# david-cortes/poismf

Measured on AMD Instinct MI355X. Metric: nonzeros/sec per full A+B sweep, higher is better.
Workload: dtype f32; 1 GPU; uniform 1000000x100000, 99949803 nnz (100000000 triplets, seed 1, duplicates summed), k=50, method=pg, maxupd=10, l2=1000, step=1e-09

## Files before the change

include/poismf_hip.h:

```cpp
#ifndef POISMF_HIP_H
#define POISMF_HIP_H

#include <stdbool.h>
#include <stddef.h>

#ifdef __cplusplus
extern "C" {
#endif

#ifdef _FOR_R
  #undef USE_FLOAT
#endif
#ifndef real_t
  #ifdef USE_FLOAT
    #define real_t float
  #else
    #define real_t double
  #endif
#endif
#ifndef sparse_ix
  #ifdef _FOR_R
    #define sparse_ix int
  #else
    #define sparse_ix size_t
// ... 211 lines not shown

POISMF_HIP_API int poismf_hip_session_decisions(poismf_hip_session *s, int which, unsigned *out, size_t nrows);
POISMF_HIP_API int poismf_hip_session_decision_stats(poismf_hip_session *s, int which, unsigned long long *out);
POISMF_HIP_API int poismf_hip_factors_multiple_decisions(real_t *A, real_t *B, real_t *Bsum, real_t *Amean, real_t *Xr,
                          sparse_ix *Xr_indptr, sparse_ix *Xr_indices, int k, size_t dimA, real_t l2_reg, real_t w_mult,
                          real_t step_size, size_t niter, size_t maxupd, int method, bool limit_step, bool reuse_mean,
                          unsigned *decisions);

POISMF_HIP_API int poismf_hip_session_colsum_blocks(poismf_hip_session *s, int which);
POISMF_HIP_API int poismf_hip_session_colsum_partial(poismf_hip_session *s, int which, int b_lo, int b_hi);
POISMF_HIP_API real_t *poismf_hip_session_partials(poismf_hip_session *s);
POISMF_HIP_API void poismf_hip_session_partials_ready(poismf_hip_session *s);

POISMF_HIP_API void poismf_hip_release_cache(void);
POISMF_HIP_API size_t poismf_hip_set_device_cache_mb(size_t mb);

POISMF_HIP_API int poismf_hip_debug_row_eval(real_t *G, double *f, real_t *B, real_t *Bsum, real_t *point, real_t *Xr,
                          sparse_ix *Xr_indptr, sparse_ix *Xr_indices, int k, size_t dimA, real_t l2_reg, real_t w_mult, int which);

POISMF_HIP_API size_t poismf_hip_debug_plan(const unsigned *row_nnz, size_t nrows, int nseg, int seg, size_t k, size_t dimF, int method,
                          size_t maxupd, real_t w_mult, int limit_step, int num_cu, char *buf, size_t cap);
POISMF_HIP_API size_t poismf_hip_debug_plan_widths(const unsigned *row_nnz, size_t nrows, int nseg, int seg, size_t k, size_t dimF, int method,
                          size_t maxupd, real_t w_mult, int limit_step, int num_cu, char *buf, size_t cap);
POISMF_HIP_API int poismf_hip_debug_lane_full_width(int full);

POISMF_HIP_API size_t poismf_hip_session_nnz(poismf_hip_session *s, int which);

#ifdef __cplusplus
}
#endif
#endif
```

poismf_amd/api.py:

```python
import ctypes as C
import os

import numpy as np

from . import build as _build
from . import harness

_METHOD = {"tncg": 1, "cg": 2, "pg": 3}
_LIBS = {}


class poismf_hip_params(C.Structure):
    pass


def _params_type(c_real):
    class Params(C.Structure):
        _fields_ = [("l2_reg", c_real), ("l1_reg", c_real), ("w_mult", c_real), ("step_size", c_real),
                    ("method", C.c_int), ("limit_step", C.c_int), ("maxupd", C.c_size_t),
                    ("early_stop", C.c_int), ("reuse_prev", C.c_int)]
    return Params


EXPORTED_SYMBOLS = (
    "run_poismf", "factors_multiple", "poismf_hip_coo_to_csr_csc", "predict_multiple", "topN", "poismf_hip_session_create", "poismf_hip_session_destroy", "poismf_hip_session_A",
    "poismf_hip_session_B", "poismf_hip_session_set_factors", "poismf_hip_session_get_factors",
    "poismf_hip_half_sweep", "poismf_hip_session_profile", "poismf_hip_session_kernel_time",
    "poismf_hip_session_nnz", "poismf_hip_selftest_log", "poismf_hip_session_eval_stats",
    "poismf_hip_session_create_coo", "poismf_hip_session_stream", "poismf_hip_session_factors_dirty", "poismf_hip_session_run",
    "poismf_hip_session_set_segments", "poismf_hip_session_segment_rows", "poismf_hip_half_sweep_segment", "poismf_hip_session_plan",
    "poismf_hip_session_launch_profile", "poismf_hip_session_decisions", "poismf_hip_session_decision_stats", "poismf_hip_factors_multiple_decisions",
    "poismf_hip_session_predict", "poismf_hip_session_topn", "poismf_hip_debug_row_eval", "poismf_hip_release_cache",
    "poismf_hip_set_device_cache_mb", "poismf_hip_session_colsum_blocks", "poismf_hip_session_colsum_partial", "poismf_hip_session_partials",
    "poismf_hip_session_partials_ready", "eval_llk", "poismf_hip_session_llk", "poismf_hip_debug_plan",
    "poismf_hip_debug_plan_widths", "poismf_hip_debug_lane_full_width",
    "poismf_hip_topn_batch", "poismf_hip_session_topn_batch", "poismf_hip_topn_batch_scratch_bytes",
    "poismf_hip_rank_batch", "poismf_hip_session_rank_batch", "poismf_hip_rank_batch_scratch_bytes",
    "poismf_hip_rank_include", "poismf_hip_session_rank_include", "poismf_hip_rank_include_scratch_bytes",
    "poismf_hip_topn_include", "poismf_hip_session_topn_include", "poismf_hip_topn_include_scratch_bytes", "poismf_hip_topn_include_slice",
    "poismf_hip_topn_shared", "poismf_hip_session_topn_shared", "poismf_hip_topn_shared_scratch_bytes",
    "poismf_hip_rank_shared", "poismf_hip_session_rank_shared", "poismf_hip_rank_shared_scratch_bytes",
    "poismf_hip_topn_deep", "poismf_hip_session_topn_deep", "poismf_hip_topn_deep_scratch_bytes",
)
TOPN_BATCH_MAX_N_TOP = 128
RANK_EXCLUDED = 0xFFFFFFFF
RANK_BATCH_MAX_ROW = 65536
RANK_BATCH_BUDGET_MB = 256
RANK_INCLUDE_SLICE = 1024
RANK_INCLUDE_GROUP = 128
TOPN_NONE = 2**64 - 1
TOPN_INCLUDE_MAX_ROW = 16777216
TOPN_SHARED_MAX_CELLS = 2**24
RANK_SHARED_CHUNK_CELLS = 2**19
TOPN_DEEP_MAX_N_TOP = 1024
TOPN_DEEP_BUDGET_MB = 1024


def load_library(use_float):
# ... 269 lines not shown
    if ret:
        raise MemoryError("Could not allocate enough memory.")
    return A, (dec[:, 0] & 0xffffff).astype(np.int64), dec[:, 1].astype(np.int64), (dec[:, 0] >> 24).astype(np.int64)


def debug_row_eval(B, Bsum, point, Xr_indptr, Xr_indices, Xr, l2_reg, w_mult=1., which=0):
    use_float = B.dtype == np.float32
    _check_arrays(use_float, (B, Bsum, point, Xr), (Xr_indptr, Xr_indices))
    lib = load_library(use_float)
    k = B.shape[1]
    n = Xr_indptr.shape[0] - 1
    G = np.empty((n, k), dtype=B.dtype)
    f = np.empty(n, dtype=np.float64)
    real = C.c_float if use_float else C.c_double
    fn = lib.poismf_hip_debug_row_eval
    fn.restype = C.c_int
    fn.argtypes = [C.c_void_p] * 8 + [C.c_int, C.c_size_t, real, real, C.c_int]
    ret = fn(_ptr(G), _ptr(f), _ptr(B), _ptr(Bsum), _ptr(point), _ptr(Xr), _ptr(Xr_indptr), _ptr(Xr_indices), k, n, l2_reg, w_mult, int(which))
    if ret:
        raise MemoryError("poismf_hip_debug_row_eval failed")
    return f, G


def debug_plan(row_nnz, k, dimF, method, use_float, nseg=1, seg=-1, maxupd=1, w_mult=1., limit_step=True, num_cu=256, widths=False):
    lib = load_library(use_float)
    row_nnz = np.ascontiguousarray(row_nnz, dtype=np.uint32)
    real = C.c_float if use_float else C.c_double
    fn = lib.poismf_hip_debug_plan_widths if widths else lib.poismf_hip_debug_plan
    fn.restype = C.c_size_t
    fn.argtypes = [C.c_void_p, C.c_size_t, C.c_int, C.c_int, C.c_size_t, C.c_size_t, C.c_int, C.c_size_t, real, C.c_int, C.c_int, C.c_void_p, C.c_size_t]
    args = (_ptr(row_nnz), len(row_nnz), int(nseg), int(seg), int(k), int(dimF), _METHOD[method], int(maxupd), w_mult, int(bool(limit_step)), int(num_cu))
    buf = C.create_string_buffer(int(fn(*args, None, 0)) + 1)
    fn(*args, buf, len(buf))
    return [(name.strip(), int(rows)) for name, rows in (item.rsplit(" rows=", 1) for item in buf.value.decode().split(";") if item.strip())]


def lane_full_width(use_float, full):
    fn = load_library(use_float).poismf_hip_debug_lane_full_width
    fn.restype, fn.argtypes = C.c_int, [C.c_int]
    return bool(fn(int(bool(full))))


class PoisMF:

    def __init__(self, k=50, method="tncg", l2_reg="auto", l1_reg=0.0, niter="auto", maxupd="auto",
                 limit_step=True, initial_step=1e-7, early_stop=True, reuse_prev=False, weight_mult=1.0,
                 random_state=1, use_float=True, handle_interrupt=True, nthreads=-1):
        assert method in ("tncg", "cg", "pg")
        self.k = int(k)
        self.method = method
        self.l2_reg_, self.maxupd_, self.niter_ = harness.auto_defaults(method, self.k, l2_reg, maxupd, niter)
        assert self.k > 0 and self.niter_ >= 1 and self.maxupd_ >= 1
        assert self.l2_reg_ >= 0. and l1_reg >= 0. and initial_step > 0. and weight_mult > 0.
        self.l1_reg_ = float(l1_reg)
        self.limit_step = bool(limit_step)
        self.initial_step = float(initial_step)
        self.early_stop = bool(early_stop)
        self.reuse_prev = bool(reuse_prev)
        self.weight_mult = float(weight_mult)
        self.random_state = random_state
        self.use_float = bool(use_float)
        self.handle_interrupt = bool(handle_interrupt)
        self.nthreads_ = 1 if nthreads < 1 else int(nthreads)
# ... 754 lines not shown
```

poismf_amd/csrc/plan.hpp:

```cpp
#pragma once
#include <hip/hip_runtime.h>

#include <algorithm>
#include <cstdio>
#include <cstdlib>

#include "../../include/poismf_hip.h"
#include "row_eval.hpp"
#include "devmem.hpp"

using namespace pmf;

inline hipError_t& pmf_last_hip_error()
{
    static thread_local hipError_t e = hipSuccess;
    return e;
}
inline void pmf_report_failure()
{
    const hipError_t e = pmf_last_hip_error();
    if (e == hipSuccess || e == hipErrorOutOfMemory) fprintf(stderr, "Error: out of memory.\n");
    else fprintf(stderr, "Error: the HIP device or runtime failed (%s) -- not an out-of-memory condition; the factors are not valid.\n", hipGetErrorString(e));
}
#define HIP_TRY(expr)                                                                              \
// ... 147 lines not shown
        if (cls <= 256) return { 2, 0, 0, 2, 1 };
        if (cls <= 512) return { 2, 0, 0, 4, 1 };
        if (cls <= 1024) return { 2, 0, 0, 8, 1 };
        if (cls <= 1536) return { 3, 0, 0, 8, 1 };
    }
    return { 0, 0, 0, 0, 0 };
}

#ifndef PMF_LANE_KU50
#if (defined(PMF_LANE_XPOSE) && PMF_LANE_XPOSE != 2) || (defined(PMF_LANE_COAL) && PMF_LANE_COAL == 0) || (defined(PMF_LANE_SPOINT) && PMF_LANE_SPOINT == 0) || \
    (defined(PMF_LANE_PK) && PMF_LANE_PK == 0) || (defined(PMF_LANE_PK_DOTS) && PMF_LANE_PK_DOTS == 0) || (defined(PMF_LANE_DIRECT) && PMF_LANE_DIRECT == 0)
#define PMF_LANE_KU50 0
#else
#define PMF_LANE_KU50 1
#endif
#endif
constexpr int LANE_KU_50 = 50;
inline int lane_used_width(size_t k, int s_load, int method, const LaneShape& ls)
{
    if (PMF_LANE_KU50 && sizeof(real_t) == 4 && method == POISMF_PG && s_load == 13 && k == (size_t)LANE_KU_50 && ls.lv == 4 && ls.waves == 4) return LANE_KU_50;
    return 0;
}

constexpr unsigned LONG_ROW_NNZ = 8192;
constexpr int LONG_NW = 8;
constexpr int SLOT_ELEMS = (int)(16 / sizeof(real_t));

int slots_per_lane(size_t k)
{
    const size_t s_load = (k * sizeof(real_t) + 15) / 16;
    return s_load <= 64 ? 1 : (s_load <= 128 ? 2 : 0);
}

}

enum class Engine {
    Reg,
    RegW,
    RegTeam,
    Lane,
    LaneTeam,
    Lds,
    LdsLong,
    Giant,
};

struct OneLaunch {
    Engine engine;
    int reg_S, nw, s_load, spl;
    int team;
    LaneShape lane;
    hipStream_t stream;
    size_t lds;
    unsigned grid, grid_mult;
    int device, num_cu;
};


int pmf_launch_one_tu1(int method, const OneLaunch& o, const HalfArgs<real_t>& a);
int pmf_launch_one_tu2(int method, const OneLaunch& o, const HalfArgs<real_t>& a);
int pmf_launch_one_tu3(int method, const OneLaunch& o, const HalfArgs<real_t>& a);
int pmf_launch_one_tu4(int method, const OneLaunch& o, const HalfArgs<real_t>& a);
int pmf_read_timing(unsigned long long* out);
```

poismf_amd/csrc/planner.hip:

```cpp
#include <algorithm>
#include <atomic>
#include <cstdio>
#include <cstdlib>
#include <cstring>
#include <functional>
#include <string>
#include <vector>

#include "session.hpp"

namespace {

unsigned length_class(unsigned n)
{
    if (n <= 256) return std::max(16u, (n + 15u) / 16u * 16u);
    if (n <= 2048) return (n + 63u) / 64u * 64u;
    unsigned cls = 4096;
    while (cls < n) cls <<= 1;
    return cls;
}

bool prefetch_enabled() { return true; }

TileGeom plan_geom(size_t k, unsigned bin_max_nnz, bool single_pass, bool want_pq)
// ... 11 lines not shown
    unsigned stream_chunk = (unsigned)(14336 / ((size_t)g.s_stride * 16)) / 16 * 16;
    stream_chunk = std::min(128u, std::max(16u, stream_chunk));
    if (!single_pass && (size_t)32 * g.s_stride * 16 <= 28 * 1024) stream_chunk = std::max(stream_chunk, 32u);
    if (!single_pass && prefetch_enabled() && ((size_t)g.s_load == (size_t)SPECIAL_SL_A || (size_t)g.s_load == (size_t)SPECIAL_SL_B))
        stream_chunk = std::max(stream_chunk, std::max(16u, (unsigned)(PMF_PRE * WAVE / g.s_load) / 16 * 16));
    unsigned cap = want;
    g.resident = 1;
    TileGeom probe = g;
    probe.cap = (int)cap;
    if (lds_bytes_per_wave(probe, sizeof(real_t)) > LDS_RESIDENT_LIMIT || (single_pass && cap > stream_chunk)) {
        cap = stream_chunk;
        probe.cap = (int)cap;
        while (cap > 16 && lds_bytes_per_wave(probe, sizeof(real_t)) > LDS_RESIDENT_LIMIT) { cap /= 2; probe.cap = (int)cap; }
        g.resident = 0;
    }
    g.cap = (int)cap;
    if (want_pq && !g.resident && (size_t)2 * bin_max_nnz * sizeof(real_t) <= 48 * 1024)
        g.pq_cap = (int)((bin_max_nnz + 15u) / 16u * 16u);
    g.prefetch = (!g.resident && prefetch_enabled()) ? 1 : 0;
    return g;
}

std::atomic<int> g_lane_full_width{0};

}

std::vector<Bin> bins_of(const unsigned* len, size_t lo, size_t hi)
{
    std::vector<Bin> bins;
    for (size_t i = lo; i < hi; i++) {
        const unsigned cls = length_class(len[i]);
        if (bins.empty() || cls != bins.back().cls) bins.push_back({ (unsigned)i, 0u, len[i], cls, 0ull });
        bins.back().count++;
        bins.back().nnz += len[i];
    }
    return bins;
}

const PlanKnobs& plan_knobs()
{
    static const PlanKnobs kn = [] {
        PlanKnobs k{};
        k.no_reg = getenv("POISMF_HIP_NO_REGTILE") != nullptr;
        k.no_team = getenv("POISMF_HIP_NO_TEAM") != nullptr; k.static_rows = getenv("POISMF_HIP_STATIC_ROWS") != nullptr;
        k.no_lane = getenv("POISMF_HIP_NO_LANE") != nullptr; k.no_lane_teams = getenv("POISMF_HIP_NO_LANE_TEAMS") != nullptr;
        k.no_giant_teams = getenv("POISMF_HIP_NO_GIANT_TEAMS") != nullptr; k.no_fork = getenv("POISMF_HIP_NO_FORK") != nullptr;
// ... 66 lines not shown
    const bool no_long = kn.longrow_nnz >= 0x40000000u;
    for (const Bin& b : bins) {
        TileGeom g = plan_geom(c.k, b.cls, c.single_pass, pm == POISMF_CG && c.limit_step);
        if (c.single_pass) { g.resident = 0; g.prefetch = prefetch_enabled() ? 1 : 0; }
        if (lane_ok) {
            LaneShape ls = lane_shape_for(b.cls, g.s_load, pm);
            if (ls.waves > 0 && g_lane_full_width.load(std::memory_order_relaxed) == 0) ls.ku = lane_used_width(c.k, g.s_load, pm, ls);
            int lane_team = 0;
            if (ls.waves == 0 && sizeof(real_t) == 8 && g.s_load == 50 && pm == POISMF_TNCG && !kn.no_lane_teams && !no_team && !kn.static_rows &&
                b.cls > 384 && b.cls <= LONG_ROW_NNZ) {
                const int m = (int)((b.cls + 383u) / 384u);
                if (m >= 2 && c.num_cu >= 2 * m) { ls = LaneShape{ 1, 0, 0, 4, 0, 32 }; lane_team = m; }
            }
            if (ls.waves > 0) {
                place(b, lane_team ? Engine::LaneTeam : Engine::Lane, g, ls.waves, 0, lane_team, ls,
                      [&](const PlannedLaunch& P) { return P.team == lane_team && P.lane == ls; });
                continue;
            }
        }
        if (reg_ok && b.cls <= reg_max) {
            const int S = reg_steps_for(ride ? b.max_nnz : b.cls);
            place(b, Engine::Reg, g, 1, S, 0, LaneShape{},
                  [&](const PlannedLaunch& P) { return P.reg_S >= S && (P.reg_S == S || (ride && b.count < 4096u)); });
            continue;
        }
        if (regw_ok && b.cls <= regw_nnz_max(pm)) {
            const int nw = regw_waves_for(b.cls, pm);
            const int S = regw_steps_for(ride ? b.max_nnz : b.cls, nw);
            place(b, Engine::RegW, g, nw, S, 0, LaneShape{},
                  [&](const PlannedLaunch& P) { return P.nw == nw && P.reg_S >= S && (P.reg_S == S || (ride && b.count < 2048u)); });
            continue;
        }
        if (team_ok) {
            const TeamShape ts = team_shape_for(b.cls);
            if (ts.members > 0) {
                place(b, Engine::RegTeam, g, TEAM_NW, ts.steps, ts.members, LaneShape{},
                      [&](const PlannedLaunch& P) { return P.team == ts.members && P.reg_S == ts.steps; });
                continue;
            }
        }
        const unsigned long_thr_here = (pm == POISMF_TNCG && !g.resident && !kn.longrow_set) ? 0u : kn.longrow_nnz;
        const TileGeom gl = long_geom(g);
        const bool long_fits = lds_bytes_per_block(gl, sizeof(real_t), LONG_NW) <= LDS_PER_CU;
        if (!no_long && long_fits && b.cls > long_thr_here) {
            const bool giant = !kn.no_giant_teams && !no_team && !kn.static_rows && pm == POISMF_TNCG && b.cls > kn.giant_nnz && c.num_cu >= 2 * GT_M;
            place(b, giant ? Engine::Giant : Engine::LdsLong, gl, LONG_NW, 0, giant ? GT_M : 0, LaneShape{}, [](const PlannedLaunch&) { return true; });
// ... 12 lines not shown
{
    const char* m = method == POISMF_PG ? "pg" : method == POISMF_EVAL ? "eval" : method == POISMF_CG ? "cg" : "tncg";
    const char* t = sizeof(real_t) == 4 ? "float" : "double";
    const LaneShape& l = L.lane;
    char txt[160] = "";
    switch (L.engine) {
        case Engine::LaneTeam: snprintf(txt, sizeof txt, "half_sweep_lane_team_kernel<%s,%s,KS=%d,V=%d,L=0+%d,NW=%d,M=%d>", t, m, L.geom.s_load, l.lv, l.lp, L.nw, L.team); break;
        case Engine::Lane:
            snprintf(txt, sizeof txt, "half_sweep_lane_kernel<%s,%s,KS=%d,V=%d,A=%d,L=%d%s,NW=%d%s%s>", t, m, L.geom.s_load, l.lv, l.la, l.ll,
                     l.lp == 32 ? "+32" : l.lp ? "+16" : "", L.nw, l.small ? ",2/SIMD" : "", l.tx == 48 ? ",TX=48" : l.tx == 64 ? ",TX=64" : "");
            break;
        case Engine::Giant: snprintf(txt, sizeof txt, "half_sweep_giant_kernel<%s,%s,NW=%d,M=%d,streamed cap=%d>", t, m, L.nw, L.team, L.geom.cap); break;
        case Engine::RegTeam: snprintf(txt, sizeof txt, "half_sweep_team_kernel<%s,%s,S=%d,NW=%d,M=%d>", t, m, L.reg_S, L.nw, L.team); break;
        case Engine::Reg: snprintf(txt, sizeof txt, "half_sweep_reg_kernel<%s,%s,S=%d>", t, m, L.reg_S); break;
        case Engine::RegW: snprintf(txt, sizeof txt, "half_sweep_regw_kernel<%s,%s,S=%d,NW=%d>", t, m, L.reg_S, L.nw); break;
        case Engine::Lds:
        case Engine::LdsLong:
            snprintf(txt, sizeof txt, "half_sweep_kernel<%s,%s,NW=%d,%s cap=%d>", t, m, L.nw, L.geom.resident ? "resident" : "streamed", L.geom.cap);
            break;
    }
    return txt;
}

std::string plan_item(int method, const PlannedLaunch& L, bool widths)
{
    std::string name = launch_name(method, L);
    if (widths && L.engine == Engine::Lane && L.lane.ku > 0) name += "[KU=" + std::to_string(L.lane.ku) + "]";
    return name + " rows=" + std::to_string(L.count) + ";";
}

std::vector<std::vector<PlannedLaunch>> plan_call(const std::vector<Half::Segment>& segs, int seg, const PlanCtx& c)
{
    std::vector<std::vector<PlannedLaunch>> passes;
    for (size_t j = 0; j < segs.size(); j++)
        if (seg < 0 || (size_t)seg == j) passes.push_back(plan_half(segs[j].bins, c));
    if (passes.empty()) passes.emplace_back();
    return passes;
}

size_t copy_text(const std::string& t, char* buf, size_t cap)
{
    if (cap > 0) {
        const size_t n = std::min(cap - 1, t.size());
        memcpy(buf, t.data(), n);
        buf[n] = 0;
    }
    return t.size();
}

static size_t debug_plan_impl(const unsigned* row_nnz, size_t nrows, int nseg, int seg, size_t k, size_t dimF, int method, size_t maxupd,
                              real_t w_mult, int limit_step, int num_cu, char* buf, size_t cap, bool widths)
{
    std::string text;
    nseg = std::max(nseg, 1);
    if (k > 0 && slots_per_lane(k) != 0 && seg < nseg) {
        std::vector<unsigned> len(row_nnz, row_nnz + nrows);
        std::vector<Half::Segment> segs;
        for (int j = 0; j < nseg; j++) {
            const size_t lo = segment_cut(nrows, j, nseg), hi = segment_cut(nrows, j + 1, nseg);
            std::stable_sort(len.begin() + lo, len.begin() + hi, std::greater<unsigned>());
            segs.push_back({ (unsigned)lo, (unsigned)hi, bins_of(len.data(), lo, hi) });
        }
        const PlanCtx c = plan_ctx(k, dimF, method, maxupd, w_mult, limit_step != 0, false, num_cu);
        for (const auto& pass : plan_call(segs, seg, c))
            for (const PlannedLaunch& L : pass) text += plan_item(method, L, widths);
    }
    return copy_text(text, buf, cap);
}

extern "C" {

size_t poismf_hip_debug_plan(const unsigned* row_nnz, size_t nrows, int nseg, int seg, size_t k, size_t dimF, int method, size_t maxupd,
                             real_t w_mult, int limit_step, int num_cu, char* buf, size_t cap)
{
    return debug_plan_impl(row_nnz, nrows, nseg, seg, k, dimF, method, maxupd, w_mult, limit_step, num_cu, buf, cap, false);
}
size_t poismf_hip_debug_plan_widths(const unsigned* row_nnz, size_t nrows, int nseg, int seg, size_t k, size_t dimF, int method, size_t maxupd,
                                    real_t w_mult, int limit_step, int num_cu, char* buf, size_t cap)
{
    return debug_plan_impl(row_nnz, nrows, nseg, seg, k, dimF, method, maxupd, w_mult, limit_step, num_cu, buf, cap, true);
}
int poismf_hip_debug_lane_full_width(int full) { return g_lane_full_width.exchange(full != 0 ? 1 : 0); }

}
```

poismf_amd/csrc/poismf_hip.hip:

```cpp
#include <hip/hip_runtime.h>

#include <algorithm>
#include <atomic>
#include <cstdio>
#include <cstdlib>
#include <type_traits>

#include "plan.hpp"
#include "reg_eval.hpp"
#include "lane_eval.hpp"
#include "solvers.hpp"

#ifndef PMF_TU
#define PMF_TU -1
#endif
constexpr bool tu_has(int kmethod) { return PMF_TU == -1 || PMF_TU == kmethod; }

template <class EV, class = void> struct cold_constants : std::false_type {};
template <class EV> struct cold_constants<EV, std::void_t<decltype(EV::COLD_CONSTANTS)>> : std::integral_constant<bool, EV::COLD_CONSTANTS> {};

template <class EV, class = void> struct has_idle_tile : std::false_type {};
template <class EV> struct has_idle_tile<EV, std::void_t<decltype(&EV::idle_tile)>> : std::true_type {};

template <class EV, class T, int NC, int METHOD>
__device__ __forceinline__ void solve_row(const HalfArgs<T>& a, EV& ev, const T (&bs)[NC], unsigned lrow, unsigned nnz)
{
    const int k = a.geom.k;
    T* out = a.M + (size_t)(a.row_offset + lrow) * (size_t)k;
    T* out_p = a.Mp != nullptr ? a.Mp + (size_t)(a.row_offset + lrow) * (size_t)a.ldM : nullptr;
    T x[NC];
    if (nnz == 0) {
        T z = (T)0;
// ... 302 lines not shown
{
    const int need = tile_regs + (method == K_PG ? PMF_PG_EXTRA : method == K_CG ? PMF_CG_EXTRA : PMF_TNC_EXTRA);
    for (int w : { 8, 6, 5, 4, 3, 2 })
        if ((512 / w) / 8 * 8 >= need) return w;
    return 1;
}
template <class T, int METHOD, int G, int NS> constexpr bool reg_pairs() { return METHOD == K_PG && sizeof(T) == 4 && G == 16 && NS == 1; }
template <class T, int METHOD, int S, int G, int NS>
__global__ __launch_bounds__(WAVE) __attribute__((amdgpu_waves_per_eu(reg_waves(4 * S * NS, METHOD)))) void half_sweep_reg_kernel(const HalfArgs<T> a)
{
    using EV = RegEval<T, S, G, NS, 1, 1, reg_pairs<T, METHOD, G, NS>()>;
    EV ev;
    constexpr int SMEM = EV::SMEM_BYTES;
    __shared__ __attribute__((aligned(16))) unsigned char smem[SMEM > 0 && METHOD == K_CG ? SMEM : 16];
#ifdef PMF_TIMING
    const unsigned long long t_kernel = __builtin_amdgcn_s_memtime();
#endif
    sweep_rows<EV, T, EV::NC, METHOD, 1>(a, ev, smem);
#ifdef PMF_TIMING
    if (ev.lane == 0) atomicAdd(&g_pmf_timing[5], __builtin_amdgcn_s_memtime() - t_kernel);
#endif
}

constexpr int regw_waves(int tile_regs, int method, int nw)
{
    const int w = reg_waves(tile_regs + (method == K_PG ? 8 : 0), method);
    return nw >= 16 && w < 4 ? 4 : (nw >= 8 && w < 2 ? 2 : w);
}
template <class T, int METHOD, int S, int G, int NS, int NW>
__global__ __launch_bounds__(WAVE* NW) __attribute__((amdgpu_waves_per_eu(regw_waves(4 * S * NS, METHOD, NW)))) void half_sweep_regw_kernel(const HalfArgs<T> a)
{
    using EV = RegEval<T, S, G, NS, NW>;
    __shared__ __attribute__((aligned(16))) unsigned char smem[EV::SMEM_BYTES];
    EV ev;
    sweep_rows<EV, T, EV::NC, METHOD, NW>(a, ev, smem);
}

template <class T, int METHOD, int S, int G, int NS, int NW, int M>
__global__ __launch_bounds__(WAVE* NW) __attribute__((amdgpu_waves_per_eu(1))) void half_sweep_team_kernel(const HalfArgs<T> a)
{
    using EV = RegEval<T, S, G, NS, NW, M>;
    constexpr int NC = EV::NC;
    __shared__ __attribute__((aligned(16))) unsigned char smem[EV::SMEM_BYTES];
    EV ev;
    ev.init(a.geom, a.F, smem);
    T bs[NC];
// ... 195 lines not shown
            if constexpr (tu_has(K_EVAL)) return launch_bin<NC, K_EVAL, SL, NW>(stream, a, lds, grid);
            else return 1;
        default:
            if constexpr (tu_has(K_TNCG)) return launch_bin<NC, K_TNCG, SL, NW>(stream, a, lds, grid);
            else return 1;
    }
}

template <int METHOD, int S, int NS> int launch_reg(hipStream_t stream, const HalfArgs<real_t>& a, unsigned grid_mult)
{
    auto kern = half_sweep_reg_kernel<real_t, METHOD, S, REG_G, NS>;
    static std::atomic<int> occ_cache{0};
    int occ = occ_cache.load(std::memory_order_relaxed);
    if (occ == 0) {
        int n = 0;
        HIP_TRY(hipOccupancyMaxActiveBlocksPerMultiprocessor(&n, reinterpret_cast<const void*>(kern), WAVE, 0));
        occ = std::max(1, n);
        occ_cache.store(occ, std::memory_order_relaxed);
    }
    const unsigned grid = (unsigned)std::min<size_t>(a.nrows, (size_t)t_num_cu * (size_t)occ * grid_mult);
    hipLaunchKernelGGL(kern, dim3(grid), dim3(WAVE), 0, stream, a);
    HIP_TRY(hipGetLastError());
    return 0;
}

template <int S, int NS> int launch_reg_method(hipStream_t stream, int method, const HalfArgs<real_t>& a, unsigned grid_mult)
{
    switch (method) {
        case POISMF_PG:
            if constexpr (tu_has(K_PG)) return launch_reg<K_PG, S, NS>(stream, a, grid_mult);
            else return 1;
        case POISMF_CG:
            if constexpr (tu_has(K_CG) && S * REG_JG <= REG_NNZ_MAX_CG && (NS == 1 || S * REG_JG <= 144)) return launch_reg<K_CG, S, NS>(stream, a, grid_mult);
            else return 1;
        case POISMF_EVAL:
            if constexpr (tu_has(K_EVAL) && S * REG_JG <= REG_NNZ_MAX_CG && (NS == 1 || S * REG_JG <= 144)) return launch_reg<K_EVAL, S, NS>(stream, a, grid_mult);
            else return 1;
        default:
            if constexpr (tu_has(K_TNCG) && S * REG_JG <= REG_NNZ_MAX_TNCG && (NS == 1 || S * REG_JG <= 112)) return launch_reg<K_TNCG, S, NS>(stream, a, grid_mult);
            else return 1;
    }
}

template <int METHOD, int S, int NS, int NW> int launch_regw(hipStream_t stream, const HalfArgs<real_t>& a, unsigned grid_mult)
{
    auto kern = half_sweep_regw_kernel<real_t, METHOD, S, REG_G, NS, NW>;
// ... 168 lines not shown
int launch_one_here(int method, const OneLaunch& o, const HalfArgs<real_t>& a)
{
    t_device = o.device; t_num_cu = o.num_cu;
    const hipStream_t st = o.stream;
    switch (o.engine) {
        case Engine::LaneTeam: return launch_lane_team(st, method, o.s_load, o.lane, a, o.grid);
        case Engine::Lane:
            switch (method) {
                case POISMF_PG: return launch_lane_shape<K_PG>(st, o.s_load, o.lane, a, o.grid_mult);
                case POISMF_CG: return launch_lane_shape<K_CG>(st, o.s_load, o.lane, a, o.grid_mult);
                case POISMF_TNCG: return launch_lane_shape<K_TNCG>(st, o.s_load, o.lane, a, o.grid_mult);
                case POISMF_EVAL: return launch_lane_shape<K_EVAL>(st, o.s_load, o.lane, a, o.grid_mult);
            }
            return 1;
#ifndef PMF_LANE_ONLY
        case Engine::RegTeam:
            if (o.team == 2 && o.reg_S == 32) return launch_team<2, 32>(st, method, a);
            if (o.team == 2 && o.reg_S == 36) return launch_team<2, 36>(st, method, a);
            if (o.team == 3 && o.reg_S == 28) return launch_team<3, 28>(st, method, a);
            if (o.team == 3 && o.reg_S == 32) return launch_team<3, 32>(st, method, a);
            if (o.team == 4 && o.reg_S == 32) return launch_team<4, 32>(st, method, a);
            return 1;
        case Engine::Reg:
            if constexpr (REG_NS_MAX == 1) return launch_reg_steps<1>(st, o.reg_S, method, a, o.grid_mult);
            else return o.s_load <= REG_G ? launch_reg_steps<1>(st, o.reg_S, method, a, o.grid_mult) : launch_reg_steps<2>(st, o.reg_S, method, a, o.grid_mult);
        case Engine::RegW:
            if constexpr (REG_G == 16) return launch_regw_steps<1>(st, o.nw, o.reg_S, method, a, o.grid_mult);
            else return o.s_load <= REG_G ? launch_regw_steps<1>(st, o.nw, o.reg_S, method, a, o.grid_mult)
                                          : launch_regw_steps<2>(st, o.nw, o.reg_S, method, a, o.grid_mult);
        case Engine::Giant:
            return with_slots(o, [&](auto nc, auto sl) { return launch_giant_method<decltype(nc)::value, decltype(sl)::value>(st, method, a, o.lds, o.grid); });
        case Engine::LdsLong:
            return with_slots(o, [&](auto nc, auto sl) { return launch_method<decltype(nc)::value, decltype(sl)::value, LONG_NW>(st, method, a, o.lds, o.grid); });
        case Engine::Lds:
            return with_slots(o, [&](auto nc, auto sl) { return launch_method<decltype(nc)::value, decltype(sl)::value>(st, method, a, o.lds, o.grid); });
#else
        default: return 1;
#endif
    }
    return 1;
}
}

#if PMF_TU == 1 || PMF_TU == -1
int pmf_launch_one_tu1(int method, const OneLaunch& o, const HalfArgs<real_t>& a) { return launch_one_here(method, o, a); }
#endif
// ... 20 lines not shown
```

poismf_amd/csrc/session.hpp:

```cpp
#pragma once
#include <string>
#include <vector>

#include "plan.hpp"

constexpr size_t LDS_RESIDENT_LIMIT = 64 * 1024;
constexpr int TEAM_LAUNCH_MAX = 32;
constexpr int TEAM_ERR_WORDS = 2 + 2 * TEAM_LAUNCH_MAX;
constexpr int MAX_LAUNCHES = 256;

struct Bin {
    unsigned begin, count;
    unsigned max_nnz;
    unsigned cls;
    unsigned long long nnz;
};

struct Half {
    size_t dimM = 0, dimF = 0;
    size_t row_begin = 0, row_end = 0;
    size_t nnz = 0;
    bool x_positive = false;
    unsigned long long* d_indptr = nullptr;
    unsigned* d_indices = nullptr;
// ... 56 lines not shown

struct PlanKnobs {
    bool no_reg, no_team, static_rows, no_lane, no_lane_teams, no_giant_teams, no_fork, no_ls_prune;
    bool longrow_set;
    unsigned longrow_nnz, giant_nnz, team_spin;
};

struct PlanCtx { size_t k, dimF, ldF; int pm; bool single_pass, limit_step, teams_off; int num_cu; };

struct PlannedLaunch : OneLaunch {
    unsigned begin, count;
    unsigned long long nnz;
    TileGeom geom;
};

inline size_t segment_cut(size_t nloc, int j, int nseg) { return nloc * (size_t)j / (size_t)nseg; }

std::vector<Bin> bins_of(const unsigned* len, size_t lo, size_t hi);
const PlanKnobs& plan_knobs();
size_t padded_row_bytes(size_t k);
PlanCtx plan_ctx(size_t k, size_t dimF, int method, size_t maxupd, real_t w_mult, bool limit_step, bool teams_off, int num_cu);
TileGeom long_geom(TileGeom g);
std::string launch_name(int method, const PlannedLaunch& L);
std::string plan_item(int method, const PlannedLaunch& L, bool widths = false);
std::vector<std::vector<PlannedLaunch>> plan_call(const std::vector<Half::Segment>& segs, int seg, const PlanCtx& c);
size_t copy_text(const std::string& t, char* buf, size_t cap);

poismf_hip_session* session_alloc(int device, void* stream, size_t dimA, size_t dimB, size_t k);
int build_half(Half& h, hipStream_t stream, const real_t* val, const sparse_ix* indptr, const sparse_ix* indices,
               size_t dimM, size_t dimF, size_t r0, size_t r1, int device = 0, HalfPending* pend = nullptr);
int finish_half_collect(Half& h, hipStream_t stream, HalfPending& pend);

int nc_for_k(size_t k);
int team_check(poismf_hip_session* s);
int half_sweep_impl(poismf_hip_session* s, int which, const poismf_hip_params* p, real_t step_size, real_t cnst_div,
                    size_t* n_unchanged, const real_t* bsum_override, real_t neg_step_override, real_t neg_step2 = (real_t)1,
                    int seg = -1);

bool interrupt_requested();
const unsigned* device_stop_word();

int run_poismf_multi(const std::vector<int>& devices, real_t* A, real_t* Xr, sparse_ix* Xr_indptr, sparse_ix* Xr_indices, real_t* B, real_t* Xc,
                     sparse_ix* Xc_indptr, sparse_ix* Xc_indices, size_t dimA, size_t dimB, size_t k, const poismf_hip_params& p, size_t numiter);
std::vector<int> devices_from_env();
```

Measured before the change: 11.47 billion nnz/s.

## Add quad-layout register engine for PG with k=50 in float

Adds a specialised Reg-engine kernel for the PG method when k=50, row stride 64 and float. Each group of four lanes splits one factor row into 12-element slices plus a 2-element tail and holds them as packed float2 values. Dot products and the gradient accumulation use packed FMAs, and cross-lane sums use DPP and ds_swizzle folds. The aim is fewer redundant loads and fewer reduction instructions per nonzero on the short-row bins. The cost is a large amount of hand-written inline assembly, a layout tied to one shape, and a dispatch that depends on a new planner flag.

```diff
diff --git a/include/poismf_hip.h b/include/poismf_hip.h
--- a/include/poismf_hip.h
+++ b/include/poismf_hip.h
@@ -257,7 +257,12 @@
                           size_t maxupd, real_t w_mult, int limit_step, int num_cu, char *buf, size_t cap);
 POISMF_HIP_API size_t poismf_hip_debug_plan_widths(const unsigned *row_nnz, size_t nrows, int nseg, int seg, size_t k, size_t dimF, int method,
                           size_t maxupd, real_t w_mult, int limit_step, int num_cu, char *buf, size_t cap);
+
+POISMF_HIP_API size_t poismf_hip_debug_plan_engines(const unsigned *row_nnz, size_t nrows, int nseg, int seg, size_t k, size_t dimF, int method,
+                          size_t maxupd, real_t w_mult, int limit_step, int num_cu, char *buf, size_t cap);
 POISMF_HIP_API int poismf_hip_debug_lane_full_width(int full);
+
+POISMF_HIP_API int poismf_hip_debug_reg_quad_off(int off);
 
 POISMF_HIP_API size_t poismf_hip_session_nnz(poismf_hip_session *s, int which);
 
diff --git a/poismf_amd/api.py b/poismf_amd/api.py
--- a/poismf_amd/api.py
+++ b/poismf_amd/api.py
@@ -33,7 +33,7 @@
     "poismf_hip_session_predict", "poismf_hip_session_topn", "poismf_hip_debug_row_eval", "poismf_hip_release_cache",
     "poismf_hip_set_device_cache_mb", "poismf_hip_session_colsum_blocks", "poismf_hip_session_colsum_partial", "poismf_hip_session_partials",
     "poismf_hip_session_partials_ready", "eval_llk", "poismf_hip_session_llk", "poismf_hip_debug_plan",
-    "poismf_hip_debug_plan_widths", "poismf_hip_debug_lane_full_width",
+    "poismf_hip_debug_plan_widths", "poismf_hip_debug_plan_engines", "poismf_hip_debug_lane_full_width", "poismf_hip_debug_reg_quad_off",
     "poismf_hip_topn_batch", "poismf_hip_session_topn_batch", "poismf_hip_topn_batch_scratch_bytes",
     "poismf_hip_rank_batch", "poismf_hip_session_rank_batch", "poismf_hip_rank_batch_scratch_bytes",
     "poismf_hip_rank_include", "poismf_hip_session_rank_include", "poismf_hip_rank_include_scratch_bytes",
@@ -349,11 +349,11 @@
     return f, G
 
 
-def debug_plan(row_nnz, k, dimF, method, use_float, nseg=1, seg=-1, maxupd=1, w_mult=1., limit_step=True, num_cu=256, widths=False):
+def debug_plan(row_nnz, k, dimF, method, use_float, nseg=1, seg=-1, maxupd=1, w_mult=1., limit_step=True, num_cu=256, widths=False, engines=False):
     lib = load_library(use_float)
     row_nnz = np.ascontiguousarray(row_nnz, dtype=np.uint32)
     real = C.c_float if use_float else C.c_double
-    fn = lib.poismf_hip_debug_plan_widths if widths else lib.poismf_hip_debug_plan
+    fn = lib.poismf_hip_debug_plan_engines if engines else lib.poismf_hip_debug_plan_widths if widths else lib.poismf_hip_debug_plan
     fn.restype = C.c_size_t
     fn.argtypes = [C.c_void_p, C.c_size_t, C.c_int, C.c_int, C.c_size_t, C.c_size_t, C.c_int, C.c_size_t, real, C.c_int, C.c_int, C.c_void_p, C.c_size_t]
     args = (_ptr(row_nnz), len(row_nnz), int(nseg), int(seg), int(k), int(dimF), _METHOD[method], int(maxupd), w_mult, int(bool(limit_step)), int(num_cu))
@@ -366,6 +366,12 @@
     fn = load_library(use_float).poismf_hip_debug_lane_full_width
     fn.restype, fn.argtypes = C.c_int, [C.c_int]
     return bool(fn(int(bool(full))))
+
+
+def reg_quad_off(use_float, off):
+    fn = load_library(use_float).poismf_hip_debug_reg_quad_off
+    fn.restype, fn.argtypes = C.c_int, [C.c_int]
+    return bool(fn(int(bool(off))))
 
 
 class PoisMF:
diff --git a/poismf_amd/csrc/plan.hpp b/poismf_amd/csrc/plan.hpp
--- a/poismf_amd/csrc/plan.hpp
+++ b/poismf_amd/csrc/plan.hpp
@@ -193,6 +193,15 @@
     return 0;
 }
 
+#ifndef PMF_REG_QUAD
+#define PMF_REG_QUAD 1
+#endif
+constexpr int QUAD_K = 50, QUAD_LD = 64;
+inline int reg_quad(size_t k, int s_load, int method, size_t ldF)
+{
+    return PMF_REG_QUAD && REG_G == 16 && sizeof(real_t) == 4 && method == POISMF_PG && s_load == 13 && k == (size_t)QUAD_K && ldF == (size_t)QUAD_LD;
+}
+
 constexpr unsigned LONG_ROW_NNZ = 8192;
 constexpr int LONG_NW = 8;
 constexpr int SLOT_ELEMS = (int)(16 / sizeof(real_t));
@@ -225,6 +234,7 @@
     size_t lds;
     unsigned grid, grid_mult;
     int device, num_cu;
+    int quad;
 };
 
 
diff --git a/poismf_amd/csrc/planner.hip b/poismf_amd/csrc/planner.hip
--- a/poismf_amd/csrc/planner.hip
+++ b/poismf_amd/csrc/planner.hip
@@ -57,6 +57,7 @@
 }
 
 std::atomic<int> g_lane_full_width{0};
+std::atomic<int> g_reg_quad_off{0};
 
 }
 
@@ -169,6 +170,7 @@
             const int S = reg_steps_for(ride ? b.max_nnz : b.cls);
             place(b, Engine::Reg, g, 1, S, 0, LaneShape{},
                   [&](const PlannedLaunch& P) { return P.reg_S >= S && (P.reg_S == S || (ride && b.count < 4096u)); });
+            launches.back().quad = g_reg_quad_off.load(std::memory_order_relaxed) == 0 ? reg_quad(c.k, g.s_load, pm, c.ldF) : 0;
             continue;
         }
         if (regw_ok && b.cls <= regw_nnz_max(pm)) {
@@ -227,10 +229,11 @@
     return txt;
 }
 
-std::string plan_item(int method, const PlannedLaunch& L, bool widths)
+std::string plan_item(int method, const PlannedLaunch& L, bool widths, bool engines)
 {
     std::string name = launch_name(method, L);
     if (widths && L.engine == Engine::Lane && L.lane.ku > 0) name += "[KU=" + std::to_string(L.lane.ku) + "]";
+    if (engines && L.engine == Engine::Reg && L.quad != 0) name += "[quad]";
     return name + " rows=" + std::to_string(L.count) + ";";
 }
 
@@ -254,7 +257,7 @@
 }
 
 static size_t debug_plan_impl(const unsigned* row_nnz, size_t nrows, int nseg, int seg, size_t k, size_t dimF, int method, size_t maxupd,
-                              real_t w_mult, int limit_step, int num_cu, char* buf, size_t cap, bool widths)
+                              real_t w_mult, int limit_step, int num_cu, char* buf, size_t cap, bool widths, bool engines = false)
 {
     std::string text;
     nseg = std::max(nseg, 1);
@@ -268,7 +271,7 @@
         }
         const PlanCtx c = plan_ctx(k, dimF, method, maxupd, w_mult, limit_step != 0, false, num_cu);
         for (const auto& pass : plan_call(segs, seg, c))
-            for (const PlannedLaunch& L : pass) text += plan_item(method, L, widths);
+            for (const PlannedLaunch& L : pass) text += plan_item(method, L, widths, engines);
     }
     return copy_text(text, buf, cap);
 }
@@ -285,6 +288,12 @@
 {
     return debug_plan_impl(row_nnz, nrows, nseg, seg, k, dimF, method, maxupd, w_mult, limit_step, num_cu, buf, cap, true);
 }
+size_t poismf_hip_debug_plan_engines(const unsigned* row_nnz, size_t nrows, int nseg, int seg, size_t k, size_t dimF, int method, size_t maxupd,
+                                     real_t w_mult, int limit_step, int num_cu, char* buf, size_t cap)
+{
+    return debug_plan_impl(row_nnz, nrows, nseg, seg, k, dimF, method, maxupd, w_mult, limit_step, num_cu, buf, cap, true, true);
+}
 int poismf_hip_debug_lane_full_width(int full) { return g_lane_full_width.exchange(full != 0 ? 1 : 0); }
-
-}
+int poismf_hip_debug_reg_quad_off(int off) { return g_reg_quad_off.exchange(off != 0 ? 1 : 0); }
+
+}
diff --git a/poismf_amd/csrc/poismf_hip.hip b/poismf_amd/csrc/poismf_hip.hip
--- a/poismf_amd/csrc/poismf_hip.hip
+++ b/poismf_amd/csrc/poismf_hip.hip
@@ -8,6 +8,7 @@
 
 #include "plan.hpp"
 #include "reg_eval.hpp"
+#include "quad_eval.hpp"
 #include "lane_eval.hpp"
 #include "solvers.hpp"
 
@@ -356,6 +357,14 @@
 #endif
 }
 
+template <int Q>
+__global__ __launch_bounds__(WAVE) __attribute__((amdgpu_waves_per_eu(reg_waves(14 * Q, K_PG)))) void half_sweep_quad_kernel(const HalfArgs<float> a)
+{
+    using EV = QuadEval<Q>;
+    EV ev;
+    sweep_rows<EV, float, EV::NC, K_PG, 1>(a, ev, nullptr);
+}
+
 constexpr int regw_waves(int tile_regs, int method, int nw)
 {
     const int w = reg_waves(tile_regs + (method == K_PG ? 8 : 0), method);
@@ -597,6 +606,35 @@
     hipLaunchKernelGGL(kern, dim3(grid), dim3(WAVE), 0, stream, a);
     HIP_TRY(hipGetLastError());
     return 0;
+}
+
+template <int Q> int launch_quad(hipStream_t stream, const HalfArgs<real_t>& a, unsigned grid_mult)
+{
+    if constexpr (tu_has(K_PG) && sizeof(real_t) == 4 && PMF_REG_QUAD != 0 && REG_G == 16 && Q >= 1 && Q <= 10) {
+        auto kern = half_sweep_quad_kernel<Q>;
+        static std::atomic<int> occ_cache{0};
+        int occ = occ_cache.load(std::memory_order_relaxed);
+        if (occ == 0) {
+            int n = 0;
+            HIP_TRY(hipOccupancyMaxActiveBlocksPerMultiprocessor(&n, reinterpret_cast<const void*>(kern), WAVE, 0));
+            occ = std::max(1, n);
+            occ_cache.store(occ, std::memory_order_relaxed);
+        }
+        const unsigned grid = (unsigned)std::min<size_t>(a.nrows, (size_t)t_num_cu * (size_t)occ * grid_mult);
+        hipLaunchKernelGGL(kern, dim3(grid), dim3(WAVE), 0, stream, a);
+        HIP_TRY(hipGetLastError());
+        return 0;
+    } else return 1;
+}
+int launch_quad_steps(hipStream_t stream, int S, int method, const HalfArgs<real_t>& a, unsigned grid_mult)
+{
+    if (method != POISMF_PG || a.geom.k != QUAD_K || a.geom.ldF != QUAD_LD) return 1;
+    switch (S) {
+#define X(NZ) case (NZ) / REG_JG: return launch_quad<(NZ) / 16>(stream, a, grid_mult);
+        PMF_REG_SIZES(X)
+#undef X
+    }
+    return 1;
 }
 
 template <int S, int NS> int launch_reg_method(hipStream_t stream, int method, const HalfArgs<real_t>& a, unsigned grid_mult)
@@ -811,6 +849,7 @@
             if (o.team == 4 && o.reg_S == 32) return launch_team<4, 32>(st, method, a);
             return 1;
         case Engine::Reg:
+            if (o.quad != 0) return launch_quad_steps(st, o.reg_S, method, a, o.grid_mult);
             if constexpr (REG_NS_MAX == 1) return launch_reg_steps<1>(st, o.reg_S, method, a, o.grid_mult);
             else return o.s_load <= REG_G ? launch_reg_steps<1>(st, o.reg_S, method, a, o.grid_mult) : launch_reg_steps<2>(st, o.reg_S, method, a, o.grid_mult);
         case Engine::RegW:
diff --git a/poismf_amd/csrc/quad_eval.hpp b/poismf_amd/csrc/quad_eval.hpp
--- /dev/null
+++ b/poismf_amd/csrc/quad_eval.hpp
@@ -0,0 +1,265 @@
+#pragma once
+#include "reg_eval.hpp"
+
+namespace pmf {
+
+#define PMF_QFOLD4(Q, A, B) \
+    "v_add_f32_dpp " Q ", " A ", " A " row_shl:4 row_mask:0xf bank_mask:0x5\n\t" \
+    "v_add_f32_dpp " Q ", " B ", " B " row_shr:4 row_mask:0xf bank_mask:0xa\n\t"
+__device__ __forceinline__ void quad_fold14(const float (&p)[14], float (&q)[7])
+{
+    asm("s_nop 1\n\t"
+        PMF_QFOLD4("%0", "%7", "%14")
+        PMF_QFOLD4("%1", "%8", "%15")
+        PMF_QFOLD4("%2", "%9", "%16")
+        PMF_QFOLD4("%3", "%10", "%17")
+        PMF_QFOLD4("%4", "%11", "%18")
+        PMF_QFOLD4("%5", "%12", "%19")
+        PMF_QFOLD4("%6", "%13", "%20")
+        : "=&v"(q[0]), "=&v"(q[1]), "=&v"(q[2]), "=&v"(q[3]), "=&v"(q[4]), "=&v"(q[5]), "=&v"(q[6])
+        : "v"(p[0]), "v"(p[1]), "v"(p[2]), "v"(p[3]), "v"(p[4]), "v"(p[5]), "v"(p[6]),
+          "v"(p[7]), "v"(p[8]), "v"(p[9]), "v"(p[10]), "v"(p[11]), "v"(p[12]), "v"(p[13]));
+}
+__device__ __forceinline__ void quad_fold7(const float (&q)[7], float (&r)[4])
+{
+    asm("s_nop 1\n\t"
+        PMF_FOLD2("row_ror:8", "0x3", "0xc", "%0", "%4", "%8")
+        PMF_FOLD2("row_ror:8", "0x3", "0xc", "%1", "%5", "%9")
+        PMF_FOLD2("row_ror:8", "0x3", "0xc", "%2", "%6", "%10")
+        PMF_FOLD1("row_ror:8", "%3", "%7")
+        : "=&v"(r[0]), "=&v"(r[1]), "=&v"(r[2]), "=&v"(r[3])
+        : "v"(q[0]), "v"(q[1]), "v"(q[2]), "v"(q[3]), "v"(q[4]), "v"(q[5]), "v"(q[6]));
+}
+
+template <int Q> struct QuadEval {
+    using T = float;
+    static_assert(Q >= 1 && Q <= 10, "one to ten steps of sixteen nonzeros");
+    typedef float V2 __attribute__((ext_vector_type(2)));
+    struct __attribute__((packed, aligned(4))) U4 { float v[4]; };
+    struct __attribute__((packed, aligned(4))) U2 { float v[2]; };
+    static constexpr int K = 50;
+    static constexpr int NP = 7;
+    static constexpr int NE = 2 * NP;
+    static constexpr int NC = 1;
+    static constexpr int NB = (Q + 3) / 4;
+    static constexpr int NW = 1, M = 1;
+    static constexpr bool PIPELINED = true;
+    static constexpr int PIPE_MW = 1;
+    static constexpr bool FUSED_SUMS = false, PREFETCH = false, MAY_CACHE = false, CACHED_GRAD = false;
+    static constexpr bool PG_LEAN = true;
+    static constexpr int SMEM_BYTES = 0;
+
+    V2 t[Q][NP];
+    V2 a[NP];
+    T xr[NB];
+    unsigned idx_n[NB];
+    const T* F;
+    unsigned zero_row;
+    int k, ldF;
+    int lane, q, wid, member;
+    int jlane;
+    int dim;
+    bool primary;
+    bool cls1, cls2, cls16, cls32;
+    int xor32_addr;
+    int quad_addr;
+    unsigned nnz;
+    unsigned n_eval;
+#ifdef PMF_PROBE
+    unsigned* probe = nullptr;
+#endif
+
+    static __host__ __device__ constexpr int acc_of(int quad)
+    {
+        const int n = ((quad >> 3) & 1) + 2 * ((quad >> 2) & 1) + 4 * ((quad >> 1) & 1);
+        return (n == 7 ? 3 : n) + 7 * (quad & 1);
+    }
+    static __host__ __device__ constexpr int quad_of(int e)
+    {
+        const int n = e % 7;
+        return (e / 7) + 2 * ((n >> 2) & 1) + 4 * ((n >> 1) & 1) + 8 * (n & 1);
+    }
+    static __host__ __device__ constexpr int dim_of(int q_, int e) { return e < 12 ? 12 * q_ + e : (q_ == 0 ? 48 + (e - 12) : -1); }
+
+    __device__ __forceinline__ void init(const TileGeom& geo, const T* F_, unsigned char*)
+    {
+        lane = lane_id();
+        F = F_;
+        k = geo.k; ldF = geo.ldF; zero_row = geo.zero_row;
+        q = lane & 3; wid = 0; member = 0;
+        jlane = 16 * q + (lane >> 2);
+        cls1 = (lane & 1) != 0; cls2 = (lane & 2) != 0; cls16 = (lane & 16) != 0; cls32 = (lane & 32) != 0;
+        const int quad = lane >> 2;
+        const int e = acc_of(quad);
+        dim = e < 12 ? 12 * q + e : (q == 0 ? 48 + (e - 12) : -1);
+        primary = dim >= 0 && (quad >> 1) != 7;
+        xor32_addr = (lane ^ 32) << 2;
+        quad_addr = q << 2;
+        asm volatile("" : "+v"(xor32_addr), "+v"(quad_addr));
+    }
+
+    __device__ __forceinline__ void load_vec(const T* p, T (&x)[NC]) const { x[0] = dim >= 0 ? p[dim >= 0 ? dim : 0] : (T)0; }
+    __device__ __forceinline__ void start_point(const T* mrow, T (&x)[NC]) const { load_vec(mrow, x); }
+    __device__ __forceinline__ void store_vec(T* p, const T (&x)[NC]) const
+    {
+        if (primary) p[dim] = x[0];
+    }
+
+    __device__ __forceinline__ void fetch_meta(const unsigned* ind, unsigned nnz_row)
+    {
+#pragma unroll
+        for (int b = 0; b < NB; b++) {
+            const unsigned j = (unsigned)(64 * b + jlane);
+            idx_n[b] = j < nnz_row ? ind[j] : zero_row;
+        }
+    }
+    __device__ __forceinline__ void begin_row(const unsigned* ind, const T* val, unsigned nnz_row)
+    {
+        fetch_meta(ind, nnz_row);
+        gather(val, nnz_row);
+    }
+    __device__ __forceinline__ unsigned* ticket_slot() const { return nullptr; }
+    __device__ __forceinline__ void gather(const T* val, unsigned nnz_row)
+    {
+        nnz = nnz_row;
+        unsigned idx[NB];
+#pragma unroll
+        for (int b = 0; b < NB; b++) {
+            const unsigned j = (unsigned)(64 * b + jlane);
+            idx[b] = idx_n[b];
+            xr[b] = j < nnz ? val[j] : (T)0;
+        }
+        const unsigned rowbytes = (unsigned)ldF * (unsigned)sizeof(T);
+        const unsigned main_off = (unsigned)q * 48u;
+        const unsigned tail_mul = q == 0 ? rowbytes : 0u;
+        const unsigned tail_off = q == 0 ? 192u : __umul24(zero_row, rowbytes);
+        static_for<0, Q>([&](auto sc) {
+            constexpr int s = decltype(sc)::value;
+            const unsigned c = group_bcast<4, s % 4>(idx[s / 4]);
+            const char* base = (const char*)F + (size_t)(__umul24(c, rowbytes) + main_off);
+            const U4 v0 = *(const U4*)base;
+            const U4 v1 = *(const U4*)(base + 16);
+            const U4 v2 = *(const U4*)(base + 32);
+            const U2 w = *(const U2*)((const char*)F + (size_t)(__umul24(c, tail_mul) + tail_off));
+            t[s][0] = (V2){ v0.v[0], v0.v[1] }; t[s][1] = (V2){ v0.v[2], v0.v[3] };
+            t[s][2] = (V2){ v1.v[0], v1.v[1] }; t[s][3] = (V2){ v1.v[2], v1.v[3] };
+            t[s][4] = (V2){ v2.v[0], v2.v[1] }; t[s][5] = (V2){ v2.v[2], v2.v[3] };
+            t[s][6] = (V2){ w.v[0], w.v[1] };
+        });
+    }
+    __device__ __forceinline__ void idle_tile()
+    {
+        asm volatile("" ::: "memory");
+#pragma unroll
+        for (int s = 0; s < Q; s++) {
+#pragma unroll
+            for (int e = 0; e < NP; e++) t[s][e] = (V2){ (T)0, (T)0 };
+        }
+    }
+
+    __device__ __forceinline__ void set_point_as_is(const T (&x)[NC])
+    {
+#define PMF_QPERM(D, E) "ds_bpermute_b32 " D ", %14, %15 offset:%" E "\n\t"
+        float r[NE];
+        asm volatile(PMF_QPERM("%0", "16") PMF_QPERM("%1", "17") PMF_QPERM("%2", "18") PMF_QPERM("%3", "19") PMF_QPERM("%4", "20")
+                     PMF_QPERM("%5", "21") PMF_QPERM("%6", "22") PMF_QPERM("%7", "23") PMF_QPERM("%8", "24") PMF_QPERM("%9", "25")
+                     PMF_QPERM("%10", "26") PMF_QPERM("%11", "27") PMF_QPERM("%12", "28") PMF_QPERM("%13", "29")
+                     "s_waitcnt lgkmcnt(0)"
+                     : "=&v"(r[0]), "=&v"(r[1]), "=&v"(r[2]), "=&v"(r[3]), "=&v"(r[4]), "=&v"(r[5]), "=&v"(r[6]), "=&v"(r[7]), "=&v"(r[8]), "=&v"(r[9]),
+                       "=&v"(r[10]), "=&v"(r[11]), "=&v"(r[12]), "=&v"(r[13])
+                     : "v"(quad_addr), "v"(x[0]), "n"(16 * quad_of(0)), "n"(16 * quad_of(1)), "n"(16 * quad_of(2)), "n"(16 * quad_of(3)),
+                       "n"(16 * quad_of(4)), "n"(16 * quad_of(5)), "n"(16 * quad_of(6)), "n"(16 * quad_of(7)), "n"(16 * quad_of(8)), "n"(16 * quad_of(9)),
+                       "n"(16 * quad_of(10)), "n"(16 * quad_of(11)), "n"(16 * quad_of(12)), "n"(16 * quad_of(13)));
+#undef PMF_QPERM
+#pragma unroll
+        for (int e = 0; e < NP; e++) a[e] = (V2){ r[2 * e], r[2 * e + 1] };
+    }
+    __device__ __forceinline__ void set_point(const T (&x)[NC]) { set_point_as_is(x); }
+
+    template <int N> __device__ __forceinline__ T quad_transpose_sum(const T (&p)[4]) const
+    {
+        T r0, r1;
+        if constexpr (N >= 2) r0 = fold_pair<0xB1>(cls1, p[0], p[1]);
+        else r0 = fold_one<0xB1>(p[0]);
+        if constexpr (N == 4) r1 = fold_pair<0xB1>(cls1, p[2], p[3]);
+        else if constexpr (N == 3) r1 = fold_one<0xB1>(p[2]);
+        if constexpr (N >= 3) return fold_pair<0x4E>(cls2, r0, r1);
+        else return fold_one<0x4E>(r0);
+    }
+
+    __device__ __forceinline__ T cross_quads(const T (&part)[NE]) const
+    {
+        T l4[7], l8[4];
+        quad_fold14(part, l4);
+        quad_fold7(l4, l8);
+        T l16[2];
+#pragma unroll
+        for (int i = 0; i < 2; i++) {
+            const T own = cls16 ? l8[i + 2] : l8[i];
+            const T send = cls16 ? l8[i] : l8[i + 2];
+            l16[i] = own + __builtin_bit_cast(T, __builtin_amdgcn_ds_swizzle(__builtin_bit_cast(int, send), 0x401f));
+        }
+        const T own = cls32 ? l16[1] : l16[0];
+        const T send = cls32 ? l16[0] : l16[1];
+        return own + __builtin_bit_cast(T, __builtin_amdgcn_ds_bpermute(xor32_addr, __builtin_bit_cast(int, send)));
+    }
+
+    template <bool WANT_F, bool WANT_G, bool FROM_CACHE = false, bool FRESH = false> __device__ __forceinline__ double eval(T sgn, T (&acc)[NC], T* = nullptr)
+    {
+        static_assert(!WANT_F && WANT_G && !FROM_CACHE, "the quad engine evaluates PG's gradient only");
+        n_eval++;
+        PMF_STAMP(*this, 0);
+        V2 part2[NP];
+        static_for<0, NB>([&](auto bc) {
+            constexpr int b = decltype(bc)::value;
+            constexpr int n = (Q - 4 * b) < 4 ? (Q - 4 * b) : 4;
+            T p[4];
+            V2 s2[n];
+#pragma unroll
+            for (int u = 0; u < n; u++) s2[u] = t[4 * b + u][0] * a[0];
+#pragma unroll
+            for (int e = 1; e < NP; e++) {
+#pragma unroll
+                for (int u = 0; u < n; u++) s2[u] = __builtin_elementwise_fma(t[4 * b + u][e], a[e], s2[u]);
+            }
+#pragma unroll
+            for (int u = 0; u < 4; u++) p[u] = u < n ? s2[u < n ? u : 0].x + s2[u < n ? u : 0].y : (T)0;
+            const T pred = quad_transpose_sum<n>(p);
+            const bool on = (unsigned)(64 * b + jlane) < nnz;
+            const T coef = on ? coef_div(sgn * xr[b], pred) : (T)0;
+            static_for<0, n>([&](auto uc) {
+                constexpr int u = decltype(uc)::value;
+                const T c = group_bcast<4, u>(coef);
+                const V2 c2 = { c, c };
+#pragma unroll
+                for (int e = 0; e < NP; e++) {
+                    if constexpr (b == 0 && u == 0) part2[e] = c2 * t[0][e];
+                    else part2[e] = __builtin_elementwise_fma(c2, t[4 * b + u][e], part2[e]);
+                }
+            });
+        });
+        PMF_STAMP(*this, 5);
+        T part[NE];
+#pragma unroll
+        for (int e = 0; e < NP; e++) { part[2 * e] = part2[e].x; part[2 * e + 1] = part2[e].y; }
+        const T g = cross_quads(part);
+        acc[0] = FRESH ? g : acc[0] + g;
+        PMF_STAMP(*this, 6);
+        return 0.0;
+    }
+
+    __device__ __forceinline__ void tile_colsum(T (&acc)[NC])
+    {
+        T part[NE];
+#pragma unroll
+        for (int i = 0; i < NE; i++) part[i] = (T)0;
+#pragma unroll
+        for (int s = 0; s < Q; s++) {
+#pragma unroll
+            for (int e = 0; e < NP; e++) { part[2 * e] += t[s][e].x; part[2 * e + 1] += t[s][e].y; }
+        }
+        acc[0] += cross_quads(part);
+    }
+};
+
+}
diff --git a/poismf_amd/csrc/session.hpp b/poismf_amd/csrc/session.hpp
--- a/poismf_amd/csrc/session.hpp
+++ b/poismf_amd/csrc/session.hpp
@@ -102,7 +102,7 @@
 PlanCtx plan_ctx(size_t k, size_t dimF, int method, size_t maxupd, real_t w_mult, bool limit_step, bool teams_off, int num_cu);
 TileGeom long_geom(TileGeom g);
 std::string launch_name(int method, const PlannedLaunch& L);
-std::string plan_item(int method, const PlannedLaunch& L, bool widths = false);
+std::string plan_item(int method, const PlannedLaunch& L, bool widths = false, bool engines = false);
 std::vector<std::vector<PlannedLaunch>> plan_call(const std::vector<Half::Segment>& segs, int seg, const PlanCtx& c);
 size_t copy_text(const std::string& t, char* buf, size_t cap);
 
```

Result: faster. 12.58 billion nnz/s, median of 6 (+9.7%).
